# stella-cv/stella_vslam

Hardware: NVIDIA H100
Metric: frames/sec (ORB+match+local BA) @1920x1080, 2000 kpts (higher is better)
Workload: dtype u8

## Files before the change

### stella_vslam_b200/csrc/lba_kernels.cu

```cuda
#include <algorithm>
#include <cmath>
#include <cstdlib>
#include <new>
#include <sched.h>

#include <chrono>
#include <memory>
#include <mutex>
#include <thread>
#include <vector>

#include "common.cuh"
#include "quat.cuh"
#include "track_chain.cuh"

namespace b200 {
namespace lba {

constexpr double kPi = 3.14159265358979323846;

struct Cam {
    int model;
    double fx, fy, cx, cy, fxb, cols, rows;
};

struct EdgeS {
    int pose;
    int pcol;
    int point;
    int lcol;
    float ox, oy, oxr;
    float inv_sigma_sq;
    float delta;
    unsigned char cam, robust, can_outlier, pad;
};


using b200::quat_normalize;
using b200::quat_to_rot;
using b200::rot_to_quat;

__device__ __forceinline__ void edge_residual(const EdgeS& e, const Cam& c, const double* Rt, const double* p, double* err, double* pc) {
    pc[0] = Rt[0] * p[0] + Rt[1] * p[1] + Rt[2] * p[2] + Rt[9];
    pc[1] = Rt[3] * p[0] + Rt[4] * p[1] + Rt[5] * p[2] + Rt[10];
    pc[2] = Rt[6] * p[0] + Rt[7] * p[1] + Rt[8] * p[2] + Rt[11];
    if (c.model == 1) {
        const double theta = atan2(pc[0], pc[2]);
        const double phi = -asin(pc[1] / sqrt(pc[0] * pc[0] + pc[1] * pc[1] + pc[2] * pc[2]));
        err[0] = (double)e.ox - c.cols * (0.5 + theta / (2 * kPi));
        err[1] = (double)e.oy - c.rows * (0.5 - phi / kPi);
        err[2] = 0.0;
    } else {
        const double rx = c.fx * pc[0] / pc[2] + c.cx;
        err[0] = (double)e.ox - rx;
        err[1] = (double)e.oy - (c.fy * pc[1] / pc[2] + c.cy);
        err[2] = (e.oxr < 0.f) ? 0.0 : (double)e.oxr - (rx - c.fxb / pc[2]);
    }
}

__device__ __forceinline__ void edge_jacobians(const EdgeS& e, const Cam& c, const double* Rt, const double* pc, double* Ji, double* Jj) {
    const double x = pc[0], y = pc[1], z = pc[2];
#pragma unroll
    for (int i = 0; i < 9; ++i) Ji[i] = 0.0;
#pragma unroll
    for (int i = 0; i < 18; ++i) Jj[i] = 0.0;
    if (c.model == 1) {
        const double L = sqrt(x * x + y * y + z * z);
        const double dx[9] = {0, z, -y, 1, 0, 0, Rt[0], Rt[1], Rt[2]};
        const double dy[9] = {-z, 0, x, 0, 1, 0, Rt[3], Rt[4], Rt[5]};
        const double dz[9] = {y, -x, 0, 0, 0, 1, Rt[6], Rt[7], Rt[8]};
        const double k0 = -(c.cols / (2 * kPi)) * (1.0 / (x * x + z * z));
        const double k1 = -(c.rows / kPi) * (1.0 / (L * sqrt(x * x + z * z)));
#pragma unroll
        for (int j = 0; j < 9; ++j) {
            const double dL = (1.0 / L) * (x * dx[j] + y * dy[j] + z * dz[j]);
            const double j0 = k0 * (z * dx[j] - x * dz[j]);
            const double j1 = k1 * (L * dy[j] - y * dL);
            if (j < 6) {
                Jj[j] = j0;
                Jj[6 + j] = j1;
            } else {
                Ji[j - 6] = j0;
                Ji[3 + j - 6] = j1;
            }
        }
        return;
    }
    const double fx = c.fx, fy = c.fy, z_sq = z * z;
#pragma unroll
    for (int j = 0; j < 3; ++j) {
        Ji[j] = -fx * Rt[j] / z + fx * x * Rt[6 + j] / z_sq;
        Ji[3 + j] = -fy * Rt[3 + j] / z + fy * y * Rt[6 + j] / z_sq;
    }
    Jj[0] = x * y / z_sq * fx; Jj[1] = -(1.0 + (x * x / z_sq)) * fx; Jj[2] = y / z * fx;
    Jj[3] = -1.0 / z * fx;     Jj[4] = 0.0;                            Jj[5] = x / z_sq * fx;
    Jj[6] = (1.0 + y * y / z_sq) * fy; Jj[7] = -x * y / z_sq * fy; Jj[8] = -x / z * fy;
    Jj[9] = 0.0;                       Jj[10] = -1.0 / z * fy;     Jj[11] = y / z_sq * fy;
    if (e.oxr >= 0.f) {
        const double fxb = c.fxb;
#pragma unroll
        for (int j = 0; j < 3; ++j) Ji[6 + j] = Ji[j] - fxb * Rt[6 + j] / z_sq;
        Jj[12] = Jj[0] - fxb * y / z_sq; Jj[13] = Jj[1] + fxb * x / z_sq; Jj[14] = Jj[2];
        Jj[15] = Jj[3];                  Jj[16] = 0.0;                    Jj[17] = Jj[5] - fxb / z_sq;
    }
}

__device__ __forceinline__ double huber_weight(double e2, double delta) { return (e2 <= delta * delta) ? 1.0 : delta / sqrt(e2); }
__device__ __forceinline__ double huber_cost(double e2, double delta) { return (e2 <= delta * delta) ? e2 : 2 * sqrt(e2) * delta - delta * delta; }

__device__ __forceinline__ double block_sum(double v, double* sh) {
    const int tid = threadIdx.x;
    sh[tid] = v;
    __syncthreads();
    for (int s = blockDim.x >> 1; s > 0; s >>= 1) {
        if (tid < s) sh[tid] += sh[tid + s];
        __syncthreads();
    }
    const double r = sh[0];
    __syncthreads();
    return r;
}


constexpr int kHplStride = 20;
__device__ __forceinline__ void ld256(const double* p, double& a, double& b, double& c, double& d) {
    const double2 lo = reinterpret_cast<const double2*>(p)[0], hi = reinterpret_cast<const double2*>(p)[1];
    a = lo.x, b = lo.y, c = hi.x, d = hi.y;
}
__device__ __forceinline__ void st256(double* p, double a, double b, double c, double d) {
    reinterpret_cast<double2*>(p)[0] = make_double2(a, b);
    reinterpret_cast<double2*>(p)[1] = make_double2(c, d);
}
__device__ __forceinline__ void load18(const double* __restrict__ p, double* out) {
    double pad0, pad1;
#pragma unroll
    for (int i = 0; i < 4; ++i) ld256(p + 4 * i, out[4 * i], out[4 * i + 1], out[4 * i + 2], out[4 * i + 3]);
    ld256(p + 16, out[16], out[17], pad0, pad1);
}

struct LmCtl {
    double lambda, ni, current_chi, last_chi, rho;
    double lambda_init, chi2[2], lambda_final[2];
    int cur, it, iterations, qmax, ok, stop_flag, round, skip_round2;
    double gain_thr;
    int outer_go;
    int need_build;
    int iters_done[2];
    int trials;
    int pad;
    const volatile int* abort_word;
};
__device__ __forceinline__ bool lm_aborted(const LmCtl* c) { return c->stop_flag || (c->abort_word && *c->abort_word); }

struct WinDev {
    int K, L, E, Kf, Lf, n, ld, n_cams;
    int lbc;
    int pad0;
    const int* e_pose;
    const int* e_point;
    const unsigned char* e_cam;
    const unsigned char* e_robust;
    const unsigned char* e_can_outlier;
    const float* e_obs;
    const float* e_isig;
    const float* e_delta;
    const int* pose_col;
    const int* pt_col;
    const Cam* cams;
    int* pt_cnt;
    int* pt_start;
    int* order;
    EdgeS* edges;
    int* epcol;
    int* pose_cnt;
    int* pose_start;
    int* pose_edges;
    int4* rowrec;
    unsigned long long* lm_mask;
    int mask_words, n_blocks;
    int* blk_cnt;
    int* blk_pair_start;
    int* blk_chunk_start;
    int4* pairs;
    struct SchurBlock* blocks;
    struct SchurChunk* chunks;
    double* chunk_part;
    int* blk_done;
    unsigned char* level;
    unsigned char* robust;
    double* q[2];
    double* t[2];
    double* Rt[2];
    double* pts[2];
    double* chi[2];
    double *Hpl, *Hll, *bl, *Dinv, *Hpp, *bp, *M, *xp;
    double *r_chi, *r_diag, *r_scale, *r_result;
    double *gP, *gD, *ginvd;
    int* fail;
    int* tickets;
    int* bad_input;
    LmCtl* ctl;
    double *qf, *tf, *pf;
    unsigned char* out;
};

__global__ void __launch_bounds__(256) plan_count_kernel(const WinDev* __restrict__ wins) {
    const WinDev& W = wins[blockIdx.y];
    const int e = blockIdx.x * blockDim.x + threadIdx.x;
    if (e >= W.E) return;
    const int p = W.e_point[e], k = W.e_pose[e];
    if (p < 0 || p >= W.L || k < 0 || k >= W.K || (int)W.e_cam[e] >= W.n_cams) {
        atomicMax(W.bad_input, e + 1);
        return;
    }
    atomicAdd(&W.pt_cnt[p], 1);
}
__global__ void __launch_bounds__(1024) plan_scan_kernel(const WinDev* __restrict__ wins) {
    const WinDev& W = wins[blockIdx.x];
    if (*W.bad_input) return;
    __shared__ int warp_sums[32];
    const int tid = threadIdx.x, lane = tid & 31, warp = tid >> 5;
    int carry = 0;
    for (int base = 0; base < W.L; base += 1024) {
        const int i = base + tid;
        const int v = i < W.L ? W.pt_cnt[i] : 0;
        int x = v;
#pragma unroll
        for (int d = 1; d < 32; d <<= 1) {
            const int y = __shfl_up_sync(0xFFFFFFFFu, x, d);
            if (lane >= d) x += y;
        }
        if (lane == 31) warp_sums[warp] = x;
        __syncthreads();
        if (warp == 0) {
            int s = warp_sums[lane];
#pragma unroll
            for (int d = 1; d < 32; d <<= 1) {
                const int y = __shfl_up_sync(0xFFFFFFFFu, s, d);
                if (lane >= d) s += y;
            }
            warp_sums[lane] = s;
        }
        __syncthreads();
        const int excl = carry + (warp ? warp_sums[warp - 1] : 0) + x - v;
        if (i < W.L) {
            W.pt_start[i] = excl;
            W.pt_cnt[i] = 0;
        }
        carry += warp_sums[31];
        __syncthreads();
    }
    if (tid == 0) W.pt_start[W.L] = carry;
}
__global__ void __launch_bounds__(256) plan_place_kernel(const WinDev* __restrict__ wins) {
    const WinDev& W = wins[blockIdx.y];
    const int e = blockIdx.x * blockDim.x + threadIdx.x;
    if (e >= W.E || *W.bad_input) return;
    const int p = W.e_point[e];
    W.order[W.pt_start[p] + atomicAdd(&W.pt_cnt[p], 1)] = e;
}
__global__ void __launch_bounds__(128) plan_sort_kernel(const WinDev* __restrict__ wins) {
    const WinDev& W = wins[blockIdx.y];
    const int l = blockIdx.x * blockDim.x + threadIdx.x;
    if (l >= W.L || *W.bad_input) return;
    const int a = W.pt_start[l], b = W.pt_start[l + 1];
    int* __restrict__ ord = W.order;
    for (int i = a + 1; i < b; ++i) {
        const int v = ord[i];
        int j = i - 1;
        while (j >= a && ord[j] > v) {
            ord[j + 1] = ord[j];
            --j;
        }
        ord[j + 1] = v;
    }
    const int lc = W.pt_col[l];
    unsigned long long* __restrict__ mask = W.lm_mask + (size_t)l * W.mask_words;
    for (int w2 = 0; w2 < W.mask_words; ++w2) mask[w2] = 0ull;
    for (int s = a; s < b; ++s) {
        const int e = ord[s];
        EdgeS d;
        d.pose = W.e_pose[e];
        d.pcol = W.pose_col[d.pose];
        d.point = l;
        d.lcol = lc;
        d.ox = W.e_obs[3 * (size_t)e];
        d.oy = W.e_obs[3 * (size_t)e + 1];
        d.oxr = W.e_obs[3 * (size_t)e + 2];
        d.inv_sigma_sq = W.e_isig[e];
        d.delta = W.e_delta[e];
// ... 233 lines not shown
            for (int i = 0; i < W.lbc; ++i) mx = fmax(mx, __ldcg(W.r_diag + i));
            for (int p = 0; p < W.Kf; ++p)
                for (int a = 0; a < 6; ++a) mx = fmax(mx, fabs(__ldcg(W.Hpp + 36 * (size_t)p + a * 7)));
            c->lambda = 1e-5 * mx;
            c->ni = 2.0;
            if (c->round == 0) c->lambda_init = c->lambda;
        }
        c->qmax = 0;
        c->rho = 0.0;
        c->need_build = 0;
        *W.fail = 0;
    }
    __syncthreads();
    compute_dinv(W, c->lambda);
}

__device__ void lm_after_trial(const WinDev& W, double* stage) {
    LmCtl* c = W.ctl;
    const double* r_result = W.r_result;
    const bool ok2 = __ldcg(r_result) != 0.0;
    const double chi_sum = ordered_sum(W.r_chi, W.lbc, stage);
    const double scale_sum = ordered_sum(W.r_scale, W.lbc, stage);
    __shared__ int s_again;
    if (threadIdx.x == 0) {
        c->trials += 1;
        const double temp_chi = ok2 ? chi_sum : 1.7976931348623157e308;
        double rho = c->current_chi - temp_chi;
        double scale = ok2 ? __ldcg(r_result + 1) + scale_sum : 0.0;
        scale += 1e-3;
        rho /= scale;
        bool broke = false;
        if (rho > 0 && isfinite(temp_chi) && ok2) {
            double alpha = 1. - pow(2 * rho - 1, 3.0);
            alpha = fmin(alpha, 2. / 3.);
            c->lambda *= fmax(1. / 3., alpha);
            c->ni = 2.0;
            c->current_chi = temp_chi;
            c->cur ^= 1;
        } else {
            c->lambda *= c->ni;
            c->ni *= 2.0;
            if (!isfinite(c->lambda)) broke = true;
        }
        if (!broke) c->qmax++;
        c->rho = rho;
        const bool again = !broke && rho < 0 && c->qmax < 10 && !lm_aborted(c);
        s_again = again ? 1 : 0;
        *W.fail = 0;
        if (!again) {
            if (c->qmax == 10 || rho == 0 || !isfinite(c->lambda)) c->ok = 0;
            const double chi_now = c->current_chi;
            if (c->it == 0) {
                c->last_chi = chi_now;
            } else {
                const double gain = (c->last_chi - chi_now) / chi_now;
                c->last_chi = chi_now;
                if (gain >= 0 && gain < c->gain_thr) c->stop_flag = 1;
            }
            c->chi2[c->round] = chi_now;
            c->lambda_final[c->round] = c->lambda;
            c->it++;
            c->iters_done[c->round] = c->it;
            c->need_build = 1;
            c->outer_go = (c->it < c->iterations && !lm_aborted(c) && c->ok) ? 1 : 0;
        }
    }
    __syncthreads();
    if (s_again) compute_dinv(W, c->lambda);
}

__device__ __forceinline__ bool last_cta_arrives(int* ticket, int n_ctas, int* smem_flag) {
    __threadfence();
    __syncthreads();
    if (threadIdx.x == 0) {
        const int t = atomicAdd(ticket, 1);
        *smem_flag = (t == n_ctas - 1);
        if (*smem_flag) *ticket = 0;
    }
    __syncthreads();
    const bool last = *smem_flag != 0;
    if (last) __threadfence();
    return last;
}

__global__ void __launch_bounds__(256) lm_round_end_kernel(const WinDev* __restrict__ wins, int round) {
    __shared__ double stage[1024];
    const WinDev& W = wins[blockIdx.x];
    LmCtl* c = W.ctl;
    if (*W.bad_input || (round == 1 && c->skip_round2)) return;
    const double chi = ordered_sum(W.r_chi, W.lbc, stage);
    if (threadIdx.x) return;
    if (c->iters_done[round] == 0) c->chi2[round] = chi;
}

enum { kBuild = 0, kTrial = 1, kRoundEnd = 2 };
constexpr int kLmThreads = 128;

template <int MODE>
__global__ void __launch_bounds__(kLmThreads, 4) landmark_kernel(const WinDev* __restrict__ wins) {
    __shared__ double sh[kLmThreads];
    const WinDev& W = wins[blockIdx.y];
    if ((int)blockIdx.x >= W.lbc) return;
    const LmCtl* ctl = W.ctl;
    if (MODE == kBuild && !(ctl->outer_go && ctl->need_build)) return;
    if (MODE == kTrial && !ctl->outer_go) return;
    if (MODE == kRoundEnd && (*W.bad_input || (ctl->round == 1 && ctl->skip_round2))) return;
    const int sidx = (ctl->cur ^ (MODE == kTrial ? 1 : 0)) & 1;
    const double* __restrict__ Rt = W.Rt[sidx];
    const double* __restrict__ pts = W.pts[sidx];
    double* __restrict__ chi = W.chi[sidx];
    const double* __restrict__ chi_carry = W.chi[sidx ^ 1];
    const int sub = threadIdx.x & 7;
    const int l = blockIdx.x * 16 + (threadIdx.x >> 3);
    const bool valid = l < W.L;
    const int a0 = valid ? W.pt_start[l] : 0, b0 = valid ? W.pt_start[l + 1] : 0;
    const int lc = valid ? W.pt_col[l] : -1;
    double cost = 0.0;
    double h[9] = {0, 0, 0, 0, 0, 0, 0, 0, 0};
    double P[3] = {0, 0, 0};
    if (valid) {
        P[0] = pts[3 * (size_t)l];
        P[1] = pts[3 * (size_t)l + 1];
        P[2] = pts[3 * (size_t)l + 2];
    }
    for (int e = a0 + sub; e < b0; e += 8) {
        const EdgeS ed = W.edges[e];
        double* __restrict__ rec = W.Hpl + (size_t)e * kHplStride;
        if (W.level[e] == 0) {
            const Cam c = W.cams[ed.cam];
            double err[3], pc[3];
            const double* T = Rt + 12 * (size_t)ed.pose;
            edge_residual(ed, c, T, P, err, pc);
            const double w = (double)ed.inv_sigma_sq;
            const double e2 = w * (err[0] * err[0] + err[1] * err[1] + err[2] * err[2]);
            chi[e] = e2;
            const bool rob = W.robust[e] != 0;
            cost += rob ? huber_cost(e2, (double)ed.delta) : e2;
            if (MODE == kBuild) {
                double Ji[9], Jj[18];
                edge_jacobians(ed, c, T, pc, Ji, Jj);
                const double ww = w * (rob ? huber_weight(e2, (double)ed.delta) : 1.0);
                const bool lfree = lc >= 0, pfree = ed.pcol >= 0;
                if (lfree) {
                    h[0] += ww * (Ji[0] * Ji[0] + Ji[3] * Ji[3] + Ji[6] * Ji[6]);
                    h[1] += ww * (Ji[0] * Ji[1] + Ji[3] * Ji[4] + Ji[6] * Ji[7]);
                    h[2] += ww * (Ji[0] * Ji[2] + Ji[3] * Ji[5] + Ji[6] * Ji[8]);
                    h[3] += ww * (Ji[1] * Ji[1] + Ji[4] * Ji[4] + Ji[7] * Ji[7]);
                    h[4] += ww * (Ji[1] * Ji[2] + Ji[4] * Ji[5] + Ji[7] * Ji[8]);
                    h[5] += ww * (Ji[2] * Ji[2] + Ji[5] * Ji[5] + Ji[8] * Ji[8]);
                    h[6] += -ww * (Ji[0] * err[0] + Ji[3] * err[1] + Ji[6] * err[2]);
                    h[7] += -ww * (Ji[1] * err[0] + Ji[4] * err[1] + Ji[7] * err[2]);
                    h[8] += -ww * (Ji[2] * err[0] + Ji[5] * err[1] + Ji[8] * err[2]);
                }
                double hp[18];
#pragma unroll
                for (int a = 0; a < 6; ++a)
#pragma unroll
                    for (int b = 0; b < 3; ++b) {
                        const double s = ww * (Jj[a] * Ji[b] + Jj[6 + a] * Ji[3 + b] + Jj[12 + a] * Ji[6 + b]);
                        hp[a * 3 + b] = (lfree && pfree) ? s : 0.0;
                    }
#pragma unroll
                for (int i = 0; i < 4; ++i) st256(rec + 4 * i, hp[4 * i], hp[4 * i + 1], hp[4 * i + 2], hp[4 * i + 3]);
                st256(rec + 16, hp[16], hp[17], 0.0, 0.0);
            }
        } else if (MODE == kBuild) {
#pragma unroll
            for (int i = 0; i < 5; ++i) st256(rec + 4 * i, 0.0, 0.0, 0.0, 0.0);
        } else if (MODE == kTrial) {
            chi[e] = chi_carry[e];
        }
    }
    if (MODE == kBuild) {
#pragma unroll
        for (int i = 0; i < 9; ++i)
#pragma unroll
            for (int s = 4; s > 0; s >>= 1) h[i] += __shfl_down_sync(0xFFFFFFFFu, h[i], s, 8);
        double mx = 0.0;
        if (valid && sub == 0 && lc >= 0) {
            const int Lf = W.Lf;
#pragma unroll
            for (int i = 0; i < 6; ++i) W.Hll[(size_t)i * Lf + lc] = h[i];
#pragma unroll
            for (int i = 0; i < 3; ++i) W.bl[(size_t)i * Lf + lc] = h[6 + i];
            mx = fmax(fabs(h[0]), fmax(fabs(h[3]), fabs(h[5])));
        }
        sh[threadIdx.x] = mx;
        __syncthreads();
        for (int s = blockDim.x >> 1; s > 0; s >>= 1) {
            if (threadIdx.x < s) sh[threadIdx.x] = fmax(sh[threadIdx.x], sh[threadIdx.x + s]);
            __syncthreads();
        }
        if (threadIdx.x == 0) W.r_diag[blockIdx.x] = sh[0];
        __syncthreads();
    }
    const double s = block_sum(cost, sh);
    if (threadIdx.x == 0) W.r_chi[blockIdx.x] = s;
    if (MODE == kTrial) {
        __shared__ int last_flag;
        __shared__ double stage[1024];
        if (!last_cta_arrives(W.tickets + 1, W.lbc, &last_flag)) return;
        lm_after_trial(W, stage);
    }
}

constexpr int kRowThreads = 256;
__global__ void __launch_bounds__(kRowThreads) pose_rows_kernel(const WinDev* __restrict__ wins) {
    const WinDev& W = wins[blockIdx.y];
    const LmCtl* ctl = W.ctl;
    if (!(ctl->outer_go && ctl->need_build)) return;
    const int n_rows = max(W.Kf, 1);
    if ((int)blockIdx.x >= n_rows) return;
    __shared__ double part[kRowThreads / 32][27];
    __shared__ int last_flag;
    __shared__ double stage[1024];
    const int tid = threadIdx.x, lane = tid & 31, warp = tid >> 5;
    if ((int)blockIdx.x < W.Kf) {
        const int i = blockIdx.x;
        const double* __restrict__ Rt = W.Rt[ctl->cur & 1];
        const double* __restrict__ pts = W.pts[ctl->cur & 1];
        const int a = W.pose_start[i], b = W.pose_start[i + 1];
        const int per = round_up(ceil_div(max(b - a, 1), kRowThreads / 32), 32);
        const int lo = a + warp * per, hi = min(b, lo + per);
        double acc[27];
#pragma unroll
        for (int x = 0; x < 27; ++x) acc[x] = 0.0;
        for (int k = lo + lane; k < hi; k += 32) {
            const int e = W.pose_edges[k];
            if (W.level[e]) continue;
            const EdgeS ed = W.edges[e];
            const Cam c = W.cams[ed.cam];
            double err[3], pc[3], Ji[9], Jj[18];
            const double* T = Rt + 12 * (size_t)ed.pose;
            edge_residual(ed, c, T, pts + 3 * (size_t)ed.point, err, pc);
            edge_jacobians(ed, c, T, pc, Ji, Jj);
            const double w = (double)ed.inv_sigma_sq;
            const double e2 = w * (err[0] * err[0] + err[1] * err[1] + err[2] * err[2]);
            const double ww = w * (W.robust[e] ? huber_weight(e2, (double)ed.delta) : 1.0);
            int t = 0;
#pragma unroll
            for (int x = 0; x < 6; ++x)
#pragma unroll
                for (int y = x; y < 6; ++y) acc[t++] += ww * (Jj[x] * Jj[y] + Jj[6 + x] * Jj[6 + y] + Jj[12 + x] * Jj[12 + y]);
#pragma unroll
            for (int x = 0; x < 6; ++x) acc[21 + x] += -ww * (Jj[x] * err[0] + Jj[6 + x] * err[1] + Jj[12 + x] * err[2]);
        }
#pragma unroll
        for (int x = 0; x < 27; ++x)
#pragma unroll
            for (int s = 16; s > 0; s >>= 1) acc[x] += __shfl_down_sync(0xFFFFFFFFu, acc[x], s);
        if (lane == 0)
#pragma unroll
            for (int x = 0; x < 27; ++x) part[warp][x] = acc[x];
        __syncthreads();
        if (tid < 27) {
            double r = 0.0;
#pragma unroll
            for (int w2 = 0; w2 < kRowThreads / 32; ++w2) r += part[w2][tid];
            if (tid < 21) {
                int x = 0, rem = tid;
                while (rem >= 6 - x) {
                    rem -= 6 - x;
                    ++x;
                }
                const int y = x + rem;
                W.Hpp[(size_t)i * 36 + x * 6 + y] = r;
                W.Hpp[(size_t)i * 36 + y * 6 + x] = r;
            } else {
                W.bp[(size_t)i * 6 + (tid - 21)] = r;
            }
        }
    }
    if (!last_cta_arrives(W.tickets, n_rows, &last_flag)) return;
    lm_after_build(W, stage);
}

__device__ __forceinline__ void dmma_m8n8k4(double& c0, double& c1, double a, double b) {
    asm volatile("mma.sync.aligned.m8n8k4.row.col.f64.f64.f64.f64 {%0,%1}, {%2}, {%3}, {%0,%1};" : "+d"(c0), "+d"(c1) : "d"(a), "d"(b));
}

__device__ __forceinline__ void schur_finish_block(const WinDev& W, const SchurBlock sb, double lambda, int lane) {
    const double* __restrict__ partials = W.chunk_part;
    double* __restrict__ M = W.M;
    const int n = W.n, ld = W.ld;
    for (int el = lane; el < 42; el += 32) {
        if (el >= 36 && sb.i != sb.j) continue;
        double sacc = 0.0;
        for (int c = sb.chunk_start; c < sb.chunk_end; ++c) sacc += __ldcg(partials + (size_t)c * 42 + el);
        if (el < 36) {
            const int r = el / 6, c = el - r * 6;
            double val = -sacc;
            if (sb.i == sb.j) val += W.Hpp[(size_t)sb.i * 36 + el] + (r == c ? lambda : 0.0);
            M[(size_t)(6 * sb.j + c) * ld + 6 * sb.i + r] = val;
            if (sb.i == sb.j) M[(size_t)(6 * sb.i + r) * ld + 6 * sb.j + c] = val;
        } else {
            const int r = el - 36;
            M[(size_t)n * ld + 6 * sb.i + r] = W.bp[(size_t)sb.i * 6 + r] - sacc;
        }
    }
}

__device__ void se3_oplus(const double* q, const double* t, const double* upd, double* qo, double* to) {
    const double* om = upd;
    const double* up = upd + 3;
    const double theta = sqrt(om[0] * om[0] + om[1] * om[1] + om[2] * om[2]);
    const double O[9] = {0, -om[2], om[1], om[2], 0, -om[0], -om[1], om[0], 0};
    double O2[9];
    for (int i = 0; i < 3; ++i)
        for (int j = 0; j < 3; ++j) O2[i * 3 + j] = O[i * 3] * O[j] + O[i * 3 + 1] * O[3 + j] + O[i * 3 + 2] * O[6 + j];
    double a, b, c, d;
    if (theta < 0.00001) {
        a = 1.0; b = 0.5; c = 0.5; d = 1.0 / 6.0;
    } else {
        a = sin(theta) / theta;
        b = (1 - cos(theta)) / (theta * theta);
        c = b;
        d = (theta - sin(theta)) / (theta * theta * theta);
    }
    double R[9], V[9];
    for (int i = 0; i < 9; ++i) {
        const double I = (i % 4 == 0) ? 1.0 : 0.0;
// ... 124 lines not shown
        }
        __syncthreads();
        PHASE(t_panel);
        const int tm = (m + 3) >> 2;
        const int n_tiles = tm * (tm + 1) / 2;
        for (int tile = tid * csize + crank; tile < n_tiles; tile += nt * csize) {
            int tr = (int)((sqrt(8.0 * tile + 1.0) - 1.0) * 0.5);
            while ((tr + 1) * (tr + 2) / 2 <= tile) ++tr;
            while (tr * (tr + 1) / 2 > tile) --tr;
            const int tc = tile - tr * (tr + 1) / 2;
            double acc[16];
#pragma unroll
            for (int a = 0; a < 16; ++a) acc[a] = 0.0;
            const int rb = tr * 4, cb = tc * 4;
#pragma unroll 4
            for (int k = 0; k < kNB; ++k) {
                const double2* pa = reinterpret_cast<const double2*>(Pn + (size_t)k * mp + rb);
                const double2* pb = reinterpret_cast<const double2*>(Pn + (size_t)k * mp + cb);
                const double2 a0 = pa[0], a1 = pa[1], b0 = pb[0], b1 = pb[1];
                const double a[4] = {a0.x, a0.y, a1.x, a1.y}, b[4] = {b0.x, b0.y, b1.x, b1.y};
#pragma unroll
                for (int u = 0; u < 4; ++u)
#pragma unroll
                    for (int w = 0; w < 4; ++w) acc[u * 4 + w] = fma(a[u], b[w], acc[u * 4 + w]);
            }
#pragma unroll
            for (int u = 0; u < 4; ++u)
#pragma unroll
                for (int w = 0; w < 4; ++w) {
                    const int r = rb + u, c = cb + w;
                    if (r < m && c <= r && r0 + c < n) M[(size_t)(r0 + r) * ld + r0 + c] -= acc[u * 4 + w];
                }
        }
        __syncthreads();
        if (csize > 1) cluster_sync_all();
        if (lead) {
            for (int idx = tid; idx < nb * nb; idx += nt) {
                const int i = idx / nb, j = idx - i * nb;
                if (j <= i) M[(size_t)(kb + i) * ld + kb + j] = D[i * (kNB + 1) + j];
            }
            for (int idx = tid; idx < m * nb; idx += nt) {
                const int t = idx / nb, j = idx - t * nb;
                M[(size_t)(r0 + t) * ld + kb + j] = Pn[(size_t)j * mp + t];
            }
        }
        __syncthreads();
        PHASE(t_trail);
    }
    if (!lead) return;
    if (bad) {
        if (tid == 0) {
            *fail = 1;
            result[0] = 0.0;
        }
    } else {
        for (int i = tid; i < n; i += nt) xs[i] = M[(size_t)n * ld + i];
        __syncthreads();
        for (int kb = ((n - 1) / kNB) * kNB; kb >= 0; kb -= kNB) {
            const int nb = min(kNB, n - kb);
            for (int idx = tid; idx < kNB * kNB; idx += nt) {
                const int i = idx / kNB, j = idx - i * kNB;
                D[i * (kNB + 1) + j] = (i < nb && j <= i) ? M[(size_t)(kb + i) * ld + kb + j] : 0.0;
            }
            __syncthreads();
            if (tid < 32) {
                double y = (tid < nb) ? xs[kb + tid] : 0.0;
#pragma unroll
                for (int j = kNB - 1; j >= 0; --j) {
                    const double xj = __shfl_sync(0xFFFFFFFFu, y, j) * ((j < nb) ? invd_all[kb + j] : 0.0);
                    if (tid == j) y = xj;
                    else if (tid < j) y = fma(-D[j * (kNB + 1) + tid], xj, y);
                }
                if (tid < nb) xs[kb + tid] = y;
            }
            __syncthreads();
            for (int i = tid; i < kb; i += nt) {
                double sacc = xs[i];
                for (int k = 0; k < nb; ++k) sacc = fma(-M[(size_t)(kb + k) * ld + i], xs[kb + k], sacc);
                xs[i] = sacc;
            }
            __syncthreads();
        }
        double sc = 0.0;
        for (int i = tid; i < n; i += nt) {
            xp[i] = xs[i];
            sc += xs[i] * (lambda * xs[i] + bp[i]);
        }
        const double tot = block_sum(sc, sh);
        PHASE(t_back);
        if (tid == 0) {
            result[0] = 1.0;
            result[1] = tot;
            result[2] = (double)t_diag;
            result[3] = (double)t_panel;
            result[4] = (double)t_trail;
            result[5] = (double)t_back;
        }
    }
#undef PHASE
    __syncthreads();
    for (int k = tid; k < K; k += nt) {
        double qn[4], tn[3];
        const int pc = pose_col[k];
        if (pc >= 0 && !bad) {
            se3_oplus(q_cur + 4 * k, t_cur + 3 * k, xs + 6 * pc, qn, tn);
        } else {
            for (int i = 0; i < 4; ++i) qn[i] = q_cur[4 * k + i];
            for (int i = 0; i < 3; ++i) tn[i] = t_cur[3 * k + i];
        }
        for (int i = 0; i < 4; ++i) q_new[4 * k + i] = qn[i];
        for (int i = 0; i < 3; ++i) t_new[3 * k + i] = tn[i];
        double R[9];
        quat_to_rot(qn, R);
        for (int i = 0; i < 9; ++i) Rt_new[12 * k + i] = R[i];
        for (int i = 0; i < 3; ++i) Rt_new[12 * k + 9 + i] = tn[i];
    }
}

constexpr int kSmmaKS = 100;
constexpr int kSmmaWarpDoubles = (6 + 7) * kSmmaKS;
__global__ void __launch_bounds__(128) schur_mma_kernel(const WinDev* __restrict__ wins) {
    extern __shared__ __align__(16) double smma[];
    const WinDev& W = wins[blockIdx.y];
    const LmCtl* ctl = W.ctl;
    if (!ctl->outer_go) return;
    const int warp = threadIdx.x >> 5, lane = threadIdx.x & 31;
    const int wid = blockIdx.x * 4 + warp;
    const int n_blocks = W.n_blocks, n_chunks = W.blk_chunk_start[n_blocks];
    if (wid >= n_chunks) {
        const int e = wid - n_chunks;
        if (e < n_blocks) {
            const SchurBlock sb = W.blocks[e];
            if (sb.chunk_start == sb.chunk_end) schur_finish_block(W, sb, ctl->lambda, lane);
        }
        return;
    }
    double* As = smma + (size_t)warp * kSmmaWarpDoubles;
    double* Bs = As + 6 * kSmmaKS;
    const SchurChunk ch = W.chunks[wid];
    const int Lf = W.Lf;
    const double* __restrict__ Hpl = W.Hpl;
    const double* __restrict__ Dinv = W.Dinv;
    const int g = lane >> 2, t4 = lane & 3;
    const double* a_row = As + min(g, 5) * kSmmaKS + t4;
    const double* b_row = Bs + min(g, 6) * kSmmaKS + t4;
    double c0 = 0.0, c1 = 0.0;
    for (int base = ch.start; base < ch.end; base += 32) {
        const int k = base + lane;
        const int np = min(32, ch.end - base);
        {
            double t[18], hc[18], b3[3];
            if (k < ch.end) {
                const int4 pr = W.pairs[k];
                double ha[18];
                load18(Hpl + (size_t)pr.x * kHplStride, ha);
                load18(Hpl + (size_t)pr.y * kHplStride, hc);
                const int lc = pr.z;
                const double D0 = Dinv[lc], D1 = Dinv[(size_t)Lf + lc], D2 = Dinv[(size_t)2 * Lf + lc];
                const double D4 = Dinv[(size_t)3 * Lf + lc], D5 = Dinv[(size_t)4 * Lf + lc], D8 = Dinv[(size_t)5 * Lf + lc];
#pragma unroll
                for (int r = 0; r < 6; ++r) {
                    t[r * 3] = ha[r * 3] * D0 + ha[r * 3 + 1] * D1 + ha[r * 3 + 2] * D2;
                    t[r * 3 + 1] = ha[r * 3] * D1 + ha[r * 3 + 1] * D4 + ha[r * 3 + 2] * D5;
                    t[r * 3 + 2] = ha[r * 3] * D2 + ha[r * 3 + 1] * D5 + ha[r * 3 + 2] * D8;
                }
                b3[0] = b3[1] = b3[2] = 0.0;
                if (ch.diag) {
                    b3[0] = W.bl[lc];
                    b3[1] = W.bl[(size_t)Lf + lc];
                    b3[2] = W.bl[(size_t)2 * Lf + lc];
                }
            } else {
#pragma unroll
                for (int i = 0; i < 18; ++i) t[i] = hc[i] = 0.0;
                b3[0] = b3[1] = b3[2] = 0.0;
            }
            double* ap = As + 3 * lane;
            double* bp2 = Bs + 3 * lane;
#pragma unroll
            for (int r = 0; r < 6; ++r)
#pragma unroll
                for (int kk = 0; kk < 3; ++kk) {
                    ap[r * kSmmaKS + kk] = t[r * 3 + kk];
                    bp2[r * kSmmaKS + kk] = hc[r * 3 + kk];
                }
#pragma unroll
            for (int kk = 0; kk < 3; ++kk) bp2[6 * kSmmaKS + kk] = b3[kk];
        }
        __syncwarp();
        const int steps = (3 * np + 3) >> 2;
#pragma unroll 4
        for (int s2 = 0; s2 < steps; ++s2) dmma_m8n8k4(c0, c1, a_row[4 * s2], b_row[4 * s2]);
        __syncwarp();
    }
    double* part = W.chunk_part + (size_t)wid * 42;
    if (g < 6) {
        if (t4 < 3) {
            part[g * 6 + 2 * t4] = c0;
            part[g * 6 + 2 * t4 + 1] = c1;
        } else {
            part[36 + g] = c0;
        }
    }
    __threadfence();
    __syncwarp();
    const SchurBlock sb = W.blocks[ch.block];
    int arrived = 0;
    if (lane == 0) arrived = atomicAdd(&W.blk_done[ch.block], 1);
    arrived = __shfl_sync(0xFFFFFFFFu, arrived, 0);
    if (arrived != sb.chunk_end - sb.chunk_start - 1) return;
    __threadfence();
    schur_finish_block(W, sb, ctl->lambda, lane);
    if (lane == 0) W.blk_done[ch.block] = 0;
}

constexpr int kCholOnChipMax = 1000;
constexpr int kCholGlobalMax = 24000;
constexpr int kGcholThreads = 256;
__global__ void __launch_bounds__(kGcholThreads) gchol_panel_kernel(const WinDev* __restrict__ wins, int kb) {
    const WinDev& W = wins[blockIdx.y];
    const LmCtl* __restrict__ ctl = W.ctl;
    const int n = W.n, ld = W.ld;
    if (!ctl->outer_go || kb >= n || *W.fail) return;
    const int nb = min(kNB, n - kb), r0 = kb + nb, m = n + 1 - r0, mp = (n + 1 + 3) & ~3;
    if ((int)blockIdx.x * kGcholThreads >= m + 4) return;
    double* __restrict__ M = W.M;
    __shared__ double D[kNB * (kNB + 1)];
    __shared__ double invd[kNB];
    __shared__ int bad;
    const int tid = threadIdx.x;
    if (tid == 0) bad = 0;
    __syncthreads();
    if (tid < 32) {
        double r[kNB];
#pragma unroll
        for (int k = 0; k < kNB; ++k) r[k] = (tid < nb && k <= tid) ? M[(size_t)(kb + tid) * ld + kb + k] : ((k == tid) ? 1.0 : 0.0);
        int b = 0;
#pragma unroll
        for (int j = 0; j < kNB; ++j) {
            const double djj = __shfl_sync(0xFFFFFFFFu, r[j], j);
            b |= (!(djj > 0.0) || !isfinite(djj)) ? 1 : 0;
            const double inv = rsqrt(djj), dd = djj * inv;
            if (tid == 0) invd[j] = inv;
            r[j] = (tid == j) ? dd : ((tid > j) ? r[j] * inv : r[j]);
            const double mine = (tid > j) ? r[j] : 0.0;
#pragma unroll
            for (int k = j + 1; k < kNB; ++k) {
                const double lkj = __shfl_sync(0xFFFFFFFFu, r[j], k);
                r[k] = fma(-((tid >= k) ? mine : 0.0), lkj, r[k]);
            }
        }
        if (tid < kNB) {
#pragma unroll
            for (int k = 0; k < kNB; ++k) D[tid * (kNB + 1) + k] = r[k];
        }
        if (tid == 0 && b) bad = 1;
    }
    __syncthreads();
    if (bad) {
        if (blockIdx.x == 0 && tid == 0) {
            *W.fail = 1;
            W.r_result[0] = 0.0;
        }
        return;
    }
    if (blockIdx.x == 0) {
        for (int idx = tid; idx < kNB * (kNB + 1); idx += kGcholThreads) W.gD[idx] = D[idx];
        if (tid < kNB && kb + tid < n) W.ginvd[kb + tid] = invd[tid];
    }
    const int t = blockIdx.x * kGcholThreads + tid;
    if (t < m) {
        const double* row = M + (size_t)(r0 + t) * ld + kb;
        double x[kNB];
#pragma unroll
        for (int j = 0; j < kNB; ++j) x[j] = (j < nb) ? row[j] : 0.0;
#pragma unroll
        for (int j = 0; j < kNB; ++j) {
            x[j] *= invd[j];
#pragma unroll
            for (int k = j + 1; k < kNB; ++k) x[k] = fma(-x[j], D[k * (kNB + 1) + j], x[k]);
        }
#pragma unroll
        for (int j = 0; j < kNB; ++j) W.gP[(size_t)j * mp + t] = x[j];
    } else if (t < min(mp, m + 4)) {
#pragma unroll
        for (int j = 0; j < kNB; ++j) W.gP[(size_t)j * mp + t] = 0.0;
    }
}

__global__ void __launch_bounds__(kGcholThreads) gchol_trail_kernel(const WinDev* __restrict__ wins, int kb) {
    const WinDev& W = wins[blockIdx.y];
    const LmCtl* __restrict__ ctl = W.ctl;
    const int n = W.n, ld = W.ld;
    if (!ctl->outer_go || kb >= n || *W.fail) return;
    const int nb = min(kNB, n - kb), r0 = kb + nb, m = n + 1 - r0, mp = (n + 1 + 3) & ~3;
    double* __restrict__ M = W.M;
    const double* __restrict__ Pn = W.gP;
    const long long gid = (long long)blockIdx.x * kGcholThreads + threadIdx.x;
    const int tm = (m + 3) >> 2;
    const long long n_tiles = (long long)tm * (tm + 1) / 2;
    if (gid < n_tiles) {
        int tr = (int)((sqrt(8.0 * (double)gid + 1.0) - 1.0) * 0.5);
        while ((long long)(tr + 1) * (tr + 2) / 2 <= gid) ++tr;
        while ((long long)tr * (tr + 1) / 2 > gid) --tr;
        const int tc = (int)(gid - (long long)tr * (tr + 1) / 2);
        double acc[16];
#pragma unroll
        for (int a = 0; a < 16; ++a) acc[a] = 0.0;
        const int rb = tr * 4, cb = tc * 4;
#pragma unroll 4
        for (int k = 0; k < kNB; ++k) {
            const double2* pa = reinterpret_cast<const double2*>(Pn + (size_t)k * mp + rb);
            const double2* pb = reinterpret_cast<const double2*>(Pn + (size_t)k * mp + cb);
            const double2 a0 = pa[0], a1 = pa[1], b0 = pb[0], b1 = pb[1];
            const double a[4] = {a0.x, a0.y, a1.x, a1.y}, b[4] = {b0.x, b0.y, b1.x, b1.y};
#pragma unroll
            for (int u = 0; u < 4; ++u)
#pragma unroll
                for (int w2 = 0; w2 < 4; ++w2) acc[u * 4 + w2] = fma(a[u], b[w2], acc[u * 4 + w2]);
        }
#pragma unroll
        for (int u = 0; u < 4; ++u)
#pragma unroll
            for (int w2 = 0; w2 < 4; ++w2) {
                const int r = rb + u, c = cb + w2;
                if (r < m && c <= r && r0 + c < n) M[(size_t)(r0 + r) * ld + r0 + c] -= acc[u * 4 + w2];
            }
    }
    const long long wb = (long long)m * nb + (long long)nb * nb;
    for (long long idx = gid; idx < wb; idx += (long long)gridDim.x * kGcholThreads) {
        if (idx < (long long)nb * nb) {
            const int i = (int)(idx / nb), j = (int)(idx - (long long)i * nb);
            if (j <= i) M[(size_t)(kb + i) * ld + kb + j] = W.gD[i * (kNB + 1) + j];
        } else {
            const long long id2 = idx - (long long)nb * nb;
            const int t = (int)(id2 / nb), j = (int)(id2 - (long long)t * nb);
            M[(size_t)(r0 + t) * ld + kb + j] = Pn[(size_t)j * mp + t];
        }
    }
}

constexpr int kGfinThreads = 1024;
__global__ void __launch_bounds__(kGfinThreads) gchol_finish_kernel(const WinDev* __restrict__ wins) {
    const WinDev& W = wins[blockIdx.x];
    const LmCtl* __restrict__ ctl = W.ctl;
    if (!ctl->outer_go) return;
    const int n = W.n, ld = W.ld, K = W.K;
    const double* __restrict__ M = W.M;
    double* __restrict__ xs = W.xp;
    const double* __restrict__ invd = W.ginvd;
    __shared__ double D[kNB * (kNB + 1)];
    __shared__ double sh[kGfinThreads];
    const int tid = threadIdx.x, nt = blockDim.x;
    const int bad = *W.fail;
    const double lambda = ctl->lambda;
    if (!bad) {
        for (int i = tid; i < n; i += nt) xs[i] = M[(size_t)n * ld + i];
        __syncthreads();
        for (int kb = ((n - 1) / kNB) * kNB; kb >= 0; kb -= kNB) {
            const int nb = min(kNB, n - kb);
            for (int idx = tid; idx < kNB * kNB; idx += nt) {
                const int i = idx / kNB, j = idx - i * kNB;
                D[i * (kNB + 1) + j] = (i < nb && j <= i) ? M[(size_t)(kb + i) * ld + kb + j] : 0.0;
            }
            __syncthreads();
            if (tid < 32) {
                double y = (tid < nb) ? xs[kb + tid] : 0.0;
#pragma unroll
                for (int j = kNB - 1; j >= 0; --j) {
                    const double xj = __shfl_sync(0xFFFFFFFFu, y, j) * ((j < nb) ? invd[kb + j] : 0.0);
                    if (tid == j) y = xj;
                    else if (tid < j) y = fma(-D[j * (kNB + 1) + tid], xj, y);
                }
                if (tid < nb) xs[kb + tid] = y;
            }
            __syncthreads();
            for (int i = tid; i < kb; i += nt) {
                double sacc = xs[i];
                for (int k = 0; k < nb; ++k) sacc = fma(-M[(size_t)(kb + k) * ld + i], xs[kb + k], sacc);
                xs[i] = sacc;
            }
            __syncthreads();
        }
        double sc = 0.0;
        for (int i = tid; i < n; i += nt) sc += xs[i] * (lambda * xs[i] + W.bp[i]);
        const double tot = block_sum(sc, sh);
        if (tid == 0) {
            W.r_result[0] = 1.0;
            W.r_result[1] = tot;
        }
    }
    __syncthreads();
    const int cur_idx = ctl->cur & 1;
    const double* __restrict__ q_cur = W.q[cur_idx];
    const double* __restrict__ t_cur = W.t[cur_idx];
    double* __restrict__ q_new = W.q[cur_idx ^ 1];
    double* __restrict__ t_new = W.t[cur_idx ^ 1];
    double* __restrict__ Rt_new = W.Rt[cur_idx ^ 1];
    for (int k = tid; k < K; k += nt) {
        double qn[4], tn[3];
        const int pc = W.pose_col[k];
        if (pc >= 0 && !bad) {
            se3_oplus(q_cur + 4 * k, t_cur + 3 * k, xs + 6 * pc, qn, tn);
        } else {
            for (int i = 0; i < 4; ++i) qn[i] = q_cur[4 * k + i];
            for (int i = 0; i < 3; ++i) tn[i] = t_cur[3 * k + i];
        }
        for (int i = 0; i < 4; ++i) q_new[4 * k + i] = qn[i];
        for (int i = 0; i < 3; ++i) t_new[3 * k + i] = tn[i];
        double R[9];
        quat_to_rot(qn, R);
        for (int i = 0; i < 9; ++i) Rt_new[12 * k + i] = R[i];
        for (int i = 0; i < 3; ++i) Rt_new[12 * k + 9 + i] = tn[i];
    }
}

__global__ void __launch_bounds__(128) backsub_kernel(const WinDev* __restrict__ wins) {
    __shared__ double sh[128];
    const WinDev& W = wins[blockIdx.y];
    const LmCtl* __restrict__ ctl = W.ctl;
    if ((int)blockIdx.x >= W.lbc || !ctl->outer_go) return;
    struct { int L, Lf; const int* pt_start; const EdgeS* edges; } v = {W.L, W.Lf, W.pt_start, W.edges};
    const double* __restrict__ Dinv = W.Dinv;
    const double* __restrict__ bl = W.bl;
    const double* __restrict__ Hpl = W.Hpl;
    const double* __restrict__ xp = W.xp;
    double* __restrict__ scale_partials = W.r_scale;
    const int* __restrict__ fail = W.fail;
    const double lambda = ctl->lambda;
    const double* __restrict__ pts_cur = W.pts[ctl->cur & 1];
    double* __restrict__ pts_new = W.pts[(ctl->cur & 1) ^ 1];
    const int sub = threadIdx.x & 7;
    const int l = blockIdx.x * 16 + (threadIdx.x >> 3);
    double sc = 0.0;
    const bool valid = l < v.L;
    const int a0 = valid ? v.pt_start[l] : 0, b0 = valid ? v.pt_start[l + 1] : 0;
    const int lc = valid ? W.pt_col[l] : -1;
    const bool solve = lc >= 0 && !*fail;
    double c0 = 0.0, c1 = 0.0, c2 = 0.0;
    if (solve) {
        for (int e = a0 + sub; e < b0; e += 8) {
            const int pcol = v.edges[e].pcol;
            if (pcol < 0) continue;
            double h[18];
            load18(Hpl + (size_t)e * kHplStride, h);
#pragma unroll
            for (int r = 0; r < 6; ++r) {
                const double x = xp[6 * pcol + r];
                c0 -= h[r * 3] * x;
                c1 -= h[r * 3 + 1] * x;
                c2 -= h[r * 3 + 2] * x;
            }
        }
    }
#pragma unroll
    for (int s = 4; s > 0; s >>= 1) {
        c0 += __shfl_down_sync(0xFFFFFFFFu, c0, s, 8);
        c1 += __shfl_down_sync(0xFFFFFFFFu, c1, s, 8);
        c2 += __shfl_down_sync(0xFFFFFFFFu, c2, s, 8);
    }
    double pn0 = 0.0, pn1 = 0.0, pn2 = 0.0;
    if (valid && sub == 0) {
        double p0 = pts_cur[3 * (size_t)l], p1 = pts_cur[3 * (size_t)l + 1], p2 = pts_cur[3 * (size_t)l + 2];
        if (solve) {
            const double bb0 = bl[lc], bb1 = bl[(size_t)v.Lf + lc], bb2 = bl[(size_t)2 * v.Lf + lc];
            c0 += bb0; c1 += bb1; c2 += bb2;
            const double D0 = Dinv[lc], D1 = Dinv[(size_t)v.Lf + lc], D2 = Dinv[(size_t)2 * v.Lf + lc];
            const double D4 = Dinv[(size_t)3 * v.Lf + lc], D5 = Dinv[(size_t)4 * v.Lf + lc], D8 = Dinv[(size_t)5 * v.Lf + lc];
            const double x0 = D0 * c0 + D1 * c1 + D2 * c2, x1 = D1 * c0 + D4 * c1 + D5 * c2, x2 = D2 * c0 + D5 * c1 + D8 * c2;
            sc = x0 * (lambda * x0 + bb0) + x1 * (lambda * x1 + bb1) + x2 * (lambda * x2 + bb2);
            p0 += x0; p1 += x1; p2 += x2;
        }
        pts_new[3 * (size_t)l] = p0; pts_new[3 * (size_t)l + 1] = p1; pts_new[3 * (size_t)l + 2] = p2;
        pn0 = p0; pn1 = p1; pn2 = p2;
    }
    const double tot = block_sum(sc, sh);
    if (threadIdx.x == 0) scale_partials[blockIdx.x] = tot;
    {
        const int base = threadIdx.x & ~7 & 31;
        pn0 = __shfl_sync(0xFFFFFFFFu, pn0, base);
        pn1 = __shfl_sync(0xFFFFFFFFu, pn1, base);
        pn2 = __shfl_sync(0xFFFFFFFFu, pn2, base);
        const int tidx = (ctl->cur & 1) ^ 1;
        const double* __restrict__ Rt = W.Rt[tidx];
        double* __restrict__ chi = W.chi[tidx];
        const double* __restrict__ chi_carry = W.chi[tidx ^ 1];
        const double P[3] = {pn0, pn1, pn2};
        double cost = 0.0;
        for (int e = a0 + sub; e < b0; e += 8) {
            if (W.level[e] == 0) {
                const EdgeS ed = v.edges[e];
                const Cam c = W.cams[ed.cam];
                double err[3], pc[3];
                edge_residual(ed, c, Rt + 12 * (size_t)ed.pose, P, err, pc);
                const double w = (double)ed.inv_sigma_sq;
                const double e2 = w * (err[0] * err[0] + err[1] * err[1] + err[2] * err[2]);
                chi[e] = e2;
                cost += W.robust[e] ? huber_cost(e2, (double)ed.delta) : e2;
            } else {
                chi[e] = chi_carry[e];
            }
        }
        __syncthreads();
        const double cs = block_sum(cost, sh);
        if (threadIdx.x == 0) W.r_chi[blockIdx.x] = cs;
        __shared__ int last_flag;
        __shared__ double stage[1024];
        if (!last_cta_arrives(W.tickets + 1, W.lbc, &last_flag)) return;
        lm_after_trial(W, stage);
    }
}

__global__ void __launch_bounds__(128) outlier_kernel(const WinDev* __restrict__ wins, int mode) {
    const WinDev& W = wins[blockIdx.y];
    const int e = blockIdx.x * blockDim.x + threadIdx.x;
    if (e >= W.E || *W.bad_input) return;
    const LmCtl* __restrict__ ctl = W.ctl;
    if (mode == 0 && ctl->skip_round2) return;
    const double* __restrict__ Rt = W.Rt[ctl->cur & 1];
    const double* __restrict__ pts = W.pts[ctl->cur & 1];
    const double* __restrict__ chi = W.chi[ctl->cur & 1];
    const EdgeS ed = W.edges[e];
    unsigned char o = 0;
    if (ed.can_outlier) {
        const double thr = (ed.oxr < 0.f) ? (double)5.99146f : (double)7.81473f;
        bool depth_ok = true;
        if (W.cams[ed.cam].model != 1) {
            const double* T = Rt + 12 * (size_t)ed.pose;
            const double* P = pts + 3 * (size_t)ed.point;
            depth_ok = 0.0 < T[6] * P[0] + T[7] * P[1] + T[8] * P[2] + T[11];
        }
        o = (thr < chi[e] || !depth_ok) ? 1 : 0;
    }
    if (mode == 0) {
        if (ed.can_outlier) {
            if (o) W.level[e] = 1;
            W.robust[e] = 0;
        }
    } else {
        W.out[W.order[e]] = o;
    }
}

__global__ void __launch_bounds__(256) lm_export_kernel(const WinDev* __restrict__ wins) {
    const WinDev& W = wins[blockIdx.y];
    const int cur = W.ctl->cur & 1;
    const int i = blockIdx.x * blockDim.x + threadIdx.x;
    if (i < 4 * W.K) W.qf[i] = W.q[cur][i];
    if (i < 3 * W.K) W.tf[i] = W.t[cur][i];
    if (i < 3 * W.L) W.pf[i] = W.pts[cur][i];
}

struct PoseEdge {
    double pw[3];
    float ox, oy, oxr, inv_sigma_sq, delta;
    int pad;
};
struct PoseProb {
    int n;
    int edge_off;
    Cam cam;
    double q[4], t[3];
};
constexpr int kPoseThreads = 256;

__device__ __forceinline__ void pose_rt(const double* q, const double* t, double* Rt) {
    quat_to_rot(q, Rt);
    Rt[9] = t[0];
    Rt[10] = t[1];
    Rt[11] = t[2];
}
template <int N>
__device__ __forceinline__ void cta_sum(double (&v)[N], double* out, double* scratch) {
    const int lane = threadIdx.x & 31, warp = threadIdx.x >> 5;
#pragma unroll
    for (int i = 0; i < N; ++i) {
#pragma unroll
        for (int s2 = 16; s2 > 0; s2 >>= 1) v[i] += __shfl_down_sync(0xFFFFFFFFu, v[i], s2);
    }
    __syncthreads();
    if (lane == 0)
#pragma unroll
        for (int i = 0; i < N; ++i) scratch[warp * N + i] = v[i];
    __syncthreads();
    if (threadIdx.x < N) {
        double r = 0.0;
        for (int w = 0; w < kPoseThreads / 32; ++w) r += scratch[w * N + threadIdx.x];
        out[threadIdx.x] = r;
    }
    __syncthreads();
}

__global__ void __launch_bounds__(kPoseThreads) pose_optimize_kernel(const PoseProb* __restrict__ probs, const PoseEdge* __restrict__ edges_all,
                                                                     unsigned char* __restrict__ level_all, unsigned char* __restrict__ flags_all,
                                                                     int trials_robust, int trials, int each_iter, double* __restrict__ pose_out,
                                                                     unsigned* __restrict__ n_valid_out) {
    __shared__ double scratch[(kPoseThreads / 32) * 28];
    __shared__ double red[28];
    __shared__ double Rt[12], Rt_trial[12], q_cur[4], t_cur[3], q_trial[4], t_trial[3], x[6];
    __shared__ double s_lambda, s_ni, s_cur_chi, s_last_chi, s_rho;
    __shared__ int s_ok2, s_go_inner, s_go_outer, s_accept, s_it, s_qmax, s_ok, s_stop, s_bad;
    const PoseProb pb = probs[blockIdx.x];
    const PoseEdge* __restrict__ edges = edges_all + pb.edge_off;
    unsigned char* __restrict__ level = level_all + pb.edge_off;
// ... 1120 lines not shown
```

Measured before the change: 9471.

## Compress Hpl records to a 3x3 block plus point, rebuilding rotation rows

Each edge's pose-landmark Hessian block is stored in compressed form: only the translational 3x3 block plus the camera-frame point (12 doubles instead of a padded 18/20). The rotational rows are rebuilt as cross products when the Schur product and back-substitution kernels read the record. This cuts Hpl memory traffic and storage by about 40% in exchange for a few extra FLOPs per load. It depends on the rotational Jacobian rows being exactly the skew-symmetric product of the translational ones, which must hold for every camera model.

```diff
diff --git a/stella_vslam_b200/csrc/lba_kernels.cu b/stella_vslam_b200/csrc/lba_kernels.cu
--- a/stella_vslam_b200/csrc/lba_kernels.cu
+++ b/stella_vslam_b200/csrc/lba_kernels.cu
@@ -122,7 +122,7 @@
 }
 
 
-constexpr int kHplStride = 20;
+constexpr int kHplStride = 12;
 __device__ __forceinline__ void ld256(const double* p, double& a, double& b, double& c, double& d) {
     const double2 lo = reinterpret_cast<const double2*>(p)[0], hi = reinterpret_cast<const double2*>(p)[1];
     a = lo.x, b = lo.y, c = hi.x, d = hi.y;
@@ -131,11 +131,22 @@
     reinterpret_cast<double2*>(p)[0] = make_double2(a, b);
     reinterpret_cast<double2*>(p)[1] = make_double2(c, d);
 }
-__device__ __forceinline__ void load18(const double* __restrict__ p, double* out) {
-    double pad0, pad1;
-#pragma unroll
-    for (int i = 0; i < 4; ++i) ld256(p + 4 * i, out[4 * i], out[4 * i + 1], out[4 * i + 2], out[4 * i + 3]);
-    ld256(p + 16, out[16], out[17], pad0, pad1);
+__device__ __forceinline__ void load_hpl_record(const double* __restrict__ p, double* out) {
+#pragma unroll
+    for (int i = 0; i < 3; ++i) ld256(p + 4 * i, out[4 * i], out[4 * i + 1], out[4 * i + 2], out[4 * i + 3]);
+}
+__device__ __forceinline__ void expand_hpl(const double* r, double* h) {
+    const double* A = r;
+    const double x = r[9], y = r[10], z = r[11];
+#pragma unroll
+    for (int b = 0; b < 3; ++b) {
+        h[b] = y * A[6 + b] - z * A[3 + b];
+        h[3 + b] = z * A[b] - x * A[6 + b];
+        h[6 + b] = x * A[3 + b] - y * A[b];
+        h[9 + b] = A[b];
+        h[12 + b] = A[3 + b];
+        h[15 + b] = A[6 + b];
+    }
 }
 
 struct LmCtl {
@@ -675,21 +686,23 @@
                     h[7] += -ww * (Ji[1] * err[0] + Ji[4] * err[1] + Ji[7] * err[2]);
                     h[8] += -ww * (Ji[2] * err[0] + Ji[5] * err[1] + Ji[8] * err[2]);
                 }
-                double hp[18];
-#pragma unroll
-                for (int a = 0; a < 6; ++a)
+                const bool both = lfree && pfree;
+                double hr[12];
+#pragma unroll
+                for (int a = 0; a < 3; ++a)
 #pragma unroll
                     for (int b = 0; b < 3; ++b) {
-                        const double s = ww * (Jj[a] * Ji[b] + Jj[6 + a] * Ji[3 + b] + Jj[12 + a] * Ji[6 + b]);
-                        hp[a * 3 + b] = (lfree && pfree) ? s : 0.0;
+                        const double s = ww * (Jj[3 + a] * Ji[b] + Jj[9 + a] * Ji[3 + b] + Jj[15 + a] * Ji[6 + b]);
+                        hr[a * 3 + b] = both ? s : 0.0;
                     }
 #pragma unroll
-                for (int i = 0; i < 4; ++i) st256(rec + 4 * i, hp[4 * i], hp[4 * i + 1], hp[4 * i + 2], hp[4 * i + 3]);
-                st256(rec + 16, hp[16], hp[17], 0.0, 0.0);
+                for (int i = 0; i < 3; ++i) hr[9 + i] = both ? pc[i] : 0.0;
+#pragma unroll
+                for (int i = 0; i < 3; ++i) st256(rec + 4 * i, hr[4 * i], hr[4 * i + 1], hr[4 * i + 2], hr[4 * i + 3]);
             }
         } else if (MODE == kBuild) {
 #pragma unroll
-            for (int i = 0; i < 5; ++i) st256(rec + 4 * i, 0.0, 0.0, 0.0, 0.0);
+            for (int i = 0; i < 3; ++i) st256(rec + 4 * i, 0.0, 0.0, 0.0, 0.0);
         } else if (MODE == kTrial) {
             chi[e] = chi_carry[e];
         }
@@ -1120,9 +1133,11 @@
             double t[18], hc[18], b3[3];
             if (k < ch.end) {
                 const int4 pr = W.pairs[k];
-                double ha[18];
-                load18(Hpl + (size_t)pr.x * kHplStride, ha);
-                load18(Hpl + (size_t)pr.y * kHplStride, hc);
+                double ra[12], rc[12], ha[18];
+                load_hpl_record(Hpl + (size_t)pr.x * kHplStride, ra);
+                load_hpl_record(Hpl + (size_t)pr.y * kHplStride, rc);
+                expand_hpl(ra, ha);
+                expand_hpl(rc, hc);
                 const int lc = pr.z;
                 const double D0 = Dinv[lc], D1 = Dinv[(size_t)Lf + lc], D2 = Dinv[(size_t)2 * Lf + lc];
                 const double D4 = Dinv[(size_t)3 * Lf + lc], D5 = Dinv[(size_t)4 * Lf + lc], D8 = Dinv[(size_t)5 * Lf + lc];
@@ -1410,14 +1425,16 @@
         for (int e = a0 + sub; e < b0; e += 8) {
             const int pcol = v.edges[e].pcol;
             if (pcol < 0) continue;
-            double h[18];
-            load18(Hpl + (size_t)e * kHplStride, h);
-#pragma unroll
-            for (int r = 0; r < 6; ++r) {
-                const double x = xp[6 * pcol + r];
-                c0 -= h[r * 3] * x;
-                c1 -= h[r * 3 + 1] * x;
-                c2 -= h[r * 3 + 2] * x;
+            double r[12];
+            load_hpl_record(Hpl + (size_t)e * kHplStride, r);
+            const double* x = xp + 6 * pcol;
+            const double w0 = x[0], w1 = x[1], w2 = x[2];
+            const double u[3] = {x[3] + (w1 * r[11] - w2 * r[10]), x[4] + (w2 * r[9] - w0 * r[11]), x[5] + (w0 * r[10] - w1 * r[9])};
+#pragma unroll
+            for (int k = 0; k < 3; ++k) {
+                c0 -= r[k * 3] * u[k];
+                c1 -= r[k * 3 + 1] * u[k];
+                c2 -= r[k * 3 + 2] * u[k];
             }
         }
     }
```

After: 10180 (median of 6 runs). 1.08x the previous value.
